# 21cmfast/21cmFAST

Hardware: AMD Instinct MI355X
Metric: IonizeBox cells/sec (512^3 HII_DIM, 40 filter radii) (higher is better)
Workload: dtype f32; 1 GPU; ComputeIonizedBox single-z, HII_DIM=512, 40 filter steps, G=2 (delta tophat + n_ion exp-MFP), first snapshot, device-resident inputs; hii_dim=512, n_radii=40, filtered_grids=2, parallelism=single GPU, fft=native

## Files before the change

### 21cmfast_amd/csrc/hip/c21hip.h

```cpp
#ifndef C21HIP_H
#define C21HIP_H

#include <stddef.h>

#include "ws_slots.h"

#ifdef __cplusplus
extern "C" {
#endif

int c21hip_device_count(void);
int c21hip_current_device(void);
int c21hip_use_device(int device);
int c21hip_is_device_ptr(const void *p);
void *c21hip_ws(int slot, size_t bytes);
__attribute__((visibility("hidden"))) const void *c21_stage_in(int slot, const void *p, size_t bytes, void *stream, int *status);
void *c21hip_ws_peek(int slot, size_t *bytes);
int c21hip_ws_adopt(int slot, void *ptr, size_t bytes);
void *c21hip_raw_alloc(size_t bytes);
void *c21hip_vmm_chunk(size_t phys_bytes, size_t map_bytes, void **va_out);
void c21hip_vmm_chunk_free(void *chunk);
int c21hip_ws_adopt_vmm(int slot, void *chunk, size_t bytes);
void c21hip_raw_free(void *p);
size_t c21hip_free_bytes(void);
// ... 59 lines not shown
                                 float R_param_a, const float *src_b, float *work_b,
                                 float *work_b2, int filter_b, float R_param_b, int nx, int ny,
                                 int nz, double box_len, double box_len_z, float R, float R2,
                                 int table_slot, int table_slot2, int phases, void *stream);
int c21hip_split_filter_x_pair1(const float *src, float *work, float *work2, int filter_type, int nx, int ny,
                                int nz, double box_len, double box_len_z, float R, float R2, int phases,
                                void *stream);
int c21hip_split_filter_xy2_pair_eval(const float *src_a, float *work_a, float *work_a2, int filter_a,
                                      const float *src_b, float *work_b, float *work_b2, int filter_b, int nx,
                                      int ny, int nz, double box_len, double box_len_z, float R, float R2,
                                      int phases, void *stream);
int c21hip_split_filter_xy_shared_pair(const float *src, float *work, float *work2,
                                       int filter_type, int nx, int ny, int nz, double box_len,
                                       double box_len_z, float R, float R2, int table_slot,
                                       int table_slot2, int phases, void *stream);
int c21hip_wev_prepare(int filter_a, float R_param_a, int filter_b, float R_param_b, int n_grids,
                       const float *R, int n_R, int nx, int ny, int nz, double box_len,
                       double box_len_z, int pair, int *enabled, void *stream);
void c21hip_wev_release(void);
int c21hip_wev_covers(void);
int c21hip_wev_applicable(int filter_a, int filter_b, int n_grids, int nx, int ny, int nz);
int c21hip_split_filter_xy_single_pair(const float *src, float *work, float *work2, int filter_type,
                                       float R_param, int nx, int ny, int nz, double box_len,
                                       double box_len_z, float R, float R2, int phases, void *stream);
typedef struct c21hip_z_ionise_desc {
    size_t size;
    const float *delta_work;
    const float *stars_work;
    const float *xe_work;
    const float *nrec_work;
    const float *nrec;
    double rec0;
    int recomb;
    float *g12;
    unsigned char *first_cross;
    unsigned *cross_plane;
    double *partials;
    double *sum_out;
    int nx, ny, nz, r_index;
    double rhocrit_omb, ion_eff;
    int mass_dep_zeta;
    double f_limit;
} c21hip_z_ionise_desc;
int c21hip_split_z_ionise(const c21hip_z_ionise_desc *desc, void *stream);
int c21hip_z_ionise_xe_supported(int nx, int ny, int nz);
int c21hip_z_ionise_recomb_supported(int nx, int ny, int nz);
int c21hip_z_ionise_recomb_xe_supported(int nx, int ny, int nz);
int c21hip_z_ionise_recomb_xe_nrec_supported(int nx, int ny, int nz);
int c21hip_z_ionise_partials(int nx, int ny, int nz);
int c21hip_split_z_sfr_gamma12(const float *sfr_work, const unsigned char *first_cross, float *g12,
                               int nx, int ny, int nz, int r_index, double g12_scale, void *stream);
int c21hip_z_xe_mask_supported(int nx, int ny, int nz);
int c21hip_split_z_xe_mask(const float *xe_work, const float *nion_dense, const double *mean_dev,
                           unsigned char *first_cross, int nx, int ny, int nz, int r_index,
                           double mean_f_coll, int fix_mean, int mass_dep_zeta, double f_limit,
                           double ion_eff, void *stream);
int c21hip_apply_first_cross_recomb(const unsigned char *first_cross, const float *R_dev,
                                    const float *prev_z_reion, int first_snapshot, double redshift,
                                    float *xH, float *z_reion, float *mfp, size_t ntot, void *stream);
int c21hip_window_tables(int table_slot, int filter_a, float R_param_a, int filter_b,
                         float R_param_b, int nx, int ny, int nz, double box_len,
                         double box_len_z, float R, void *stream);
int c21hip_split_z_c2r_minmax(const float *split_work, float *real_out, long out_zstride, int nx,
                              int ny, int nz, double *partials, double *minmax_out, void *stream);
int c21hip_z_table_band_supported(int nx, int ny, int nz);
int c21hip_split_z_minmax_only(const float *split_work, int nx, int ny, int nz, double *partials,
// ... 10 lines not shown
                             double *partials, double *stats_out, void *stream);
int c21hip_batched_stats(const double *partials, long stride, int nb, int count,
                         double *stats_out, void *stream);
int c21hip_floor_scale_stats(const float *in, long in_zstride, float *out, int nx, int ny, int nz,
                             double min_value, double const_factor, double *partials,
                             double *stats_out, void *stream);
int c21hip_split_z_c2r_div(const float *split_work, float *real_out, long out_zstride, int nx,
                           int ny, int nz, float divisor, void *stream);
int c21hip_split_z_c2r_out(const float *split_work, float *real_out, long out_zstride, int nx,
                           int ny, int nz, float scale, float divisor, int floor_density,
                           void *stream);
int c21hip_split_xblock_log2(int nx);
int c21hip_split_kop(const float *in_split, float *out_split, int nx, int ny, int nz,
                     double box_len, double box_len_z, int axis0, int axis1, void *stream);
int c21hip_split_sepop_xy(const float *split_src, float *split_work, int nx, int ny, int nz,
                          double box_len, double box_len_z, int axis0, int axis1, void *stream);
int c21hip_split_fold(const float *hi_split, float *lo_split, int nx, int ny, int nz, int f,
                      double box_len, double box_len_z, int axis0, int axis1, void *stream);
int c21hip_split_fold_multi(const float *hi_split, float *const lo_split[4], const int ops[4], int n_out, int nx,
                            int ny, int nz, int f, double box_len, double box_len_z, float tophat_R, void *stream);
int c21hip_lpt2_source(const float *const diag[3], const float *const off[3], float *out, size_t n,
                       float norm, void *stream);
int c21hip_copy_filter_split(const float *src_split, float *dst_split, int nx, int ny, int nz,
                             double box_len, double box_len_z, int filter_type, float R,
                             float R_param, int apply, void *stream);
int c21hip_split_z_c2r(const float *split_work, float *real_out, long out_zstride, int nx, int ny,
                       int nz, void *stream);
int c21hip_batched_means(const double *partials, long stride, int n_partials, int first, int step,
                         int count, double ntot, int mass_dep_zeta, double f_limit, double *sums,
                         double *means, void *stream);
int c21hip_z_cross_bits_supported(int nx, int ny, int nz);
int c21hip_resolve_crossings(const unsigned *bits, int r_hi, int r_lo, unsigned char *first_cross,
                             size_t nlines, void *stream);
int c21hip_split_filter_xy_shared(const float *src, float *work, int filter_type, int nx, int ny,
                                  int nz, double box_len, double box_len_z, float R, int apply,
                                  int table_slot, void *stream);
int c21hip_bench_pass(int kind, int n, int filter_a, int filter_b, float R, float R_param_b,
                      double box_len, int reps, void *stream, float *ms_out);
int c21hip_reduce_sum(const double *partials, int n, double *out, void *stream);
int c21hip_reduce_op(const double *partials, int n, int op, double *stage, double *out,
                     void *stream);

int c21hip_pack_clip(const float *dense, float *padded, int nx, int ny, int nz, double factor,
                     double lo, double hi, void *stream);
int c21hip_unpack_scale(const float *padded, float *dense, int nx, int ny, int nz, float scale,
                        void *stream);
int c21hip_divide_inplace(float *buf, size_t n, float divisor, void *stream);
int c21hip_divide_inplace_f64(float *buf, size_t n, double divisor, void *stream);
int c21hip_fill(float *buf, size_t n, float value, void *stream);
int c21hip_add_scalar(float *buf, size_t n, float value, void *stream);
int c21hip_widen(const float *in, double *out, size_t n, void *stream);

int c21hip_copy_filter(const float *src_c, float *dst_c, int nx, int ny, int nz, double box_len,
                       double box_len_z, int filter_type, float R, float R_param, int apply,
                       void *stream);
int c21hip_copy_filter_star(const float *src_c, float *dst_c, int nx, int ny, int nz,
                            double box_len, double box_len_z, int filter_type, float R,
                            float R_param, float R_star, int apply, void *stream);

typedef struct c21_gsl_stream_desc {
    unsigned long long out_offset;
    unsigned long long count;
    unsigned int kind;
    unsigned int state_offset;
} c21_gsl_stream_desc;
#define C21_GSL_HDR 8
// ... 537 lines not shown
```

### 21cmfast_amd/csrc/hip/fft_native.hip

```cpp
#include <hip/hip_runtime.h>

#include <cmath>
#include <map>
#include <mutex>
#include <vector>

#include "c21hip.h"
#include "fcoll_device.h"
#include "ms_window.h"
#include "c21cm_abi.h"
#include "c21cm_grid.h"

#ifndef C21X_XPAIR_THREADS
#define C21X_XPAIR_THREADS 512
#endif
#ifndef C21X_ZW_TSRC_OCC
#define C21X_ZW_TSRC_OCC 1
#endif
#ifndef C21X_ZW_BLOCK
#define C21X_ZW_BLOCK 256
#endif

namespace {
constexpr int kBlock = 256;
constexpr int TZ = 16;
constexpr int line_tile_cols(int n) { return n == 1536 ? TZ / 2 : TZ; }
template <int N>
__device__ __forceinline__ int fft_out_row(int g) {
    return (N >= 1024) ? ((g & 1) ? N / 2 + (g >> 1) : (g >> 1)) : g;
}

#ifndef C21X_XB_MIN
#define C21X_XB_MIN 1024
#endif
#ifndef C21X_XB_LOG2
#define C21X_XB_LOG2 3
#endif
__host__ __device__ constexpr int split_xb_log2(int nx) { return nx >= C21X_XB_MIN ? C21X_XB_LOG2 : 0; }
__host__ __device__ __forceinline__ long logical_line(long m, int ny, int lb) {
    if (lb == 0) return m;
    const long blk = (long)ny << lb;
    const long xbk = m / blk, rem = m - xbk * blk;
    const long y = rem >> lb, xi = rem & ((1 << lb) - 1);
    return ((xbk << lb) + xi) * ny + y;
}

#define LAUNCH_CHECK()                                                                  \
    do {                                                                                \
        hipError_t e_ = hipGetLastError();                                              \
        if (e_ != hipSuccess) {                                                         \
            c21hip_set_error("kernel launch failed: %s (%s:%d)", hipGetErrorString(e_), \
                             __FILE__, __LINE__);                                       \
            return C21CM_IO_ERROR;                                                      \
        }                                                                               \
    } while (0)

#include "fft_device.h"

template <int N, int COLS, int ROW, int R, int SIGN, bool LAST, int THREADS>
__device__ __forceinline__ void stockham_stage(float2 *tile, const float2 *tw, int log2s) {
    constexpr int NB = N / R;
    constexpr int ITEMS = NB * COLS;
    constexpr int kBlock = THREADS;
    constexpr int PER = (ITEMS + kBlock - 1) / kBlock;
    float2 v[PER][R];
#pragma unroll
    for (int u = 0; u < PER; u++) {
        const int i = threadIdx.x + kBlock * u;
        if (ITEMS % kBlock == 0 || i < ITEMS) {
            const int col = i % COLS, b = i / COLS;
#pragma unroll
// ... 1510 lines not shown
    __syncthreads();
    fft_tile<H, LZ, ZROW, -1, kBlock>(tile, twH);
    constexpr int NPRE = (H / 2 + 1) * LZ;
    for (int i = threadIdx.x; i < NPRE; i += kBlock) {
        const int li = i % LZ, k = i / LZ;
        if (k == 0) {
            const float2 z0 = tile[li];
            tile[li] = make_float2(z0.x + z0.y, 0.f);
            a.nyq[logical_line(l0 + li, a.ny, a.lb)] = make_float2(z0.x - z0.y, 0.f);
        } else {
            const float2 A = tile[k * ZROW + li], B = tile[(H - k) * ZROW + li];
            const float2 E = make_float2(0.5f * (A.x + B.x), 0.5f * (A.y - B.y));
            const float2 D = make_float2(0.5f * (A.x - B.x), 0.5f * (A.y + B.y));
            const float2 wD = cmul(D, twN[k]);
            tile[k * ZROW + li] = make_float2(E.x + wD.y, E.y - wD.x);
            tile[(H - k) * ZROW + li] = make_float2(E.x - wD.y, -E.y - wD.x);
        }
    }
    __syncthreads();
#pragma unroll
    for (int u = 0; u < NIN; u++) {
        const int f = threadIdx.x + kBlock * u;
        const int li = f / H, k = f % H;
        a.main[(l0 + li) * H + k] = tile[k * ZROW + li];
    }
}

struct ZFusedArgs {
    const float2 *d_main, *d_nyq;
    const float2 *s_main, *s_nyq;
    const float2 *x_main, *x_nyq;
    unsigned char *first_cross;
    unsigned *cross_bits;
    double *partials;
    double rhocrit_omb, ion_eff, f_limit;
    int mass_dep_zeta, r_index;
    int ny, lb;
    int store_all;
    int reverse;
    int rc;
    const float *nrec;
    double rec0;
    int x_is_nrec;
    const float2 *n_main, *n_nyq;
    float *g12;
};

template <int NZ>
__global__ void __launch_bounds__(kBlock)
z_c2r_ionise_kernel(ZFusedArgs a, const float2 *__restrict__ twH_global,
                    const float2 *__restrict__ twN_global) {
    constexpr int H = NZ / 2, LZ = LZ_FUSED, ZROW = LZ + 1;
    constexpr int NOUT = ZGeom<NZ, LZ>::NOUT;
    extern __shared__ float4 lds_raw[];
    float2 *tile = reinterpret_cast<float2 *>(lds_raw);
    float2 *twH = tile + H * ZROW;
    float2 *twN = twH + H;
    for (int t = threadIdx.x; t < H; t += kBlock) twH[t] = twH_global[t];
    for (int t = threadIdx.x; t <= H / 2; t += kBlock) twN[t] = twN_global[t];

    const long l0 = (long)blockIdx.x * LZ;
    float4 reg_d[ZGeom<NZ, LZ>::NLOAD], reg_s[ZGeom<NZ, LZ>::NLOAD];
    z_issue_loads<NZ, LZ>(a.d_main, l0, reg_d);
    z_issue_loads<NZ, LZ>(a.s_main, l0, reg_s);
    uchar2 old[NOUT];
#pragma unroll
// ... 473 lines not shown
            f1 = a.mass_dep_zeta && floor_lhs * opd1 > (opd1 + r1) * n1;
        }
        const bool i0 = (!RC && floor_ionises) || f0 || ((double)s0 * a.ion_eff > D0);
        const bool i1 = (!RC && floor_ionises) || f1 || ((double)s1 * a.ion_eff > D1);
        if constexpr (CB) {
            cb |= (i0 ? (1u << q) : 0u) | (i1 ? (0x10000u << q) : 0u);
            continue;
        }
        uchar2 m = MASK16 ? reinterpret_cast<const uchar2 *>(L)[j]
                          : (EARLY ? old[(EARLY && !MASK16) ? q : 0] : reinterpret_cast<const uchar2 *>(mrow)[j]);
        const bool n0 = i0 && m.x == 0, n1 = i1 && m.y == 0;
        if (n0) m.x = (unsigned char)a.r_index;
        if (n1) m.y = (unsigned char)a.r_index;
        if constexpr (MASK16) {
            if (n0 || n1) reinterpret_cast<uchar2 *>(L)[j] = m;
        } else if (n0 || n1 || a.store_all)
            reinterpret_cast<uchar2 *>(mrow)[j] = m;
        if constexpr (RC) {
            float *grow = a.g12 + lline * NZ + 2 * j;
            if (n0 && a.rc != 2) grow[0] = fmaxf(xd[q].x, dmin);
            if (n1 && a.rc != 2) grow[1] = fmaxf(xd[q].y, dmin);
        }
        if constexpr (TS && RC) __builtin_amdgcn_sched_barrier(0);
    }
    if constexpr (MASK16) {
        wave_fence();
#pragma unroll
        for (int v = 0; v < MV; v++) {
            const uint4 n = reinterpret_cast<const uint4 *>(L)[b * MV + v], o = mreg[v];
            if (a.store_all || n.x != o.x || n.y != o.y || n.z != o.z || n.w != o.w)
                reinterpret_cast<uint4 *>(mrow)[b * MV + v] = n;
        }
    }
    if constexpr (CB) a.cross_bits[lline * (NZ / 32) + b] = cb;
#pragma unroll
    for (int off = 32; off > 0; off >>= 1) acc += __shfl_down(acc, off, 64);
    if (lane == 0) red[wave] = acc;
    __syncthreads();
    if (threadIdx.x == 0) {
        double sum = 0.;
#pragma unroll
        for (int w = 0; w < ZBLK / 64; w++) sum += red[w];
        a.partials[blk] = sum;
    }
}

template <int A, int EPI, int P = 16>
__global__ void __launch_bounds__(kBlock)
zw_c2r_kernel(ZPassArgs a, const float2 *__restrict__ twH_global,
              const float2 *__restrict__ twN_global) {
    constexpr int H = P * A, NZ = 2 * H, ZWL = zw_lines(P);
    constexpr int LINE_LDS = A * (P + 1) + 4;
    static_assert(LINE_LDS % 2 == 0, "16-byte aligned line regions (EPI 7)");
    __shared__ __attribute__((aligned(16))) float2 lines[ZWL * LINE_LDS];
    __shared__ float2 twH[H], twN[H];
    for (int t = threadIdx.x; t < H; t += kBlock) {
        twH[t] = twH_global[t];
        twN[t] = twN_global[t];
    }
    const int lane = threadIdx.x & 63, wave = threadIdx.x >> 6;
    const int g = lane / P, b = lane % P;
    const int lw = wave * (64 / P) + g;
    const unsigned blk = a.reverse ? gridDim.x - 1 - blockIdx.x : blockIdx.x;
    const long line = (long)blk * ZWL + lw;
    float2 *L = lines + lw * LINE_LDS;
    const float2 *src = a.main + line * H;
    float2 x[A];
// ... 1747 lines not shown
}

extern "C" int c21hip_split_z_ionise(const c21hip_z_ionise_desc *d, void *stream) {
    if (!d || d->size != sizeof(*d)) {
        c21hip_set_error("fused pass Z: the descriptor's size member is not sizeof(c21hip_z_ionise_desc)");
        return C21CM_VALUE_ERROR;
    }
    if (d->cross_plane && !c21hip_z_cross_bits_supported(d->nx, d->ny, d->nz)) {
        c21hip_set_error("fused pass Z: crossing bits are not available for this grid");
        return C21CM_VALUE_ERROR;
    }
    const long nlines = (long)d->nx * d->ny;
    const long n_main = nlines * (d->nz / 2);
    const ZFusedWant w{d->xe_work != nullptr, d->recomb != 0, d->recomb && d->nrec_work, d->cross_plane != nullptr};
    ZFusedArgs a{};
    a.ny = d->ny;
    a.lb = split_xb_log2(d->nx);
    a.d_main = reinterpret_cast<const float2 *>(d->delta_work);
    a.d_nyq = a.d_main + n_main;
    a.s_main = reinterpret_cast<const float2 *>(d->stars_work);
    a.s_nyq = a.s_main + n_main;
    const float *third = w.xe ? d->xe_work : (w.nrec ? d->nrec_work : nullptr);
    if (third) {
        a.x_main = reinterpret_cast<const float2 *>(third);
        a.x_nyq = a.x_main + n_main;
    }
    if (w.xe && w.nrec) {
        a.n_main = reinterpret_cast<const float2 *>(d->nrec_work);
        a.n_nyq = a.n_main + n_main;
    } else
        a.x_is_nrec = w.nrec;
    a.first_cross = d->first_cross;
    a.cross_bits = d->cross_plane;
    a.partials = d->partials;
    a.rhocrit_omb = d->rhocrit_omb;
    a.ion_eff = d->ion_eff;
    a.f_limit = d->f_limit;
    a.mass_dep_zeta = d->mass_dep_zeta;
    a.r_index = d->r_index;
    if (w.rc) {
#ifdef C21CM_DIAG_BUILD
        a.rc = getenv("C21CM_DIAG_RC_NOSTORE") ? 2 : 1;
#else
        a.rc = 1;
#endif
        a.g12 = d->g12;
        if (!w.nrec) {
            a.nrec = d->nrec;
            a.rec0 = d->rec0;
        }
        a.reverse = 1;
    } else {
        static const int store_all = [] {
            const char *e = getenv("C21CM_MASK_STORE_ALL");
            return (e && e[0] == '1') ? 1 : 0;
        }();
        a.store_all = store_all;
        static const int reverse = [] {
            const char *e = getenv("C21CM_ZREV");
            return (e && e[0] == '0') ? 0 : 1;
        }();
        a.reverse = reverse;
    }
    int n_partials = 0;
    const int st = dispatch_z_fused(d->nz, a, w, nlines, (hipStream_t)stream, &n_partials);
    if (st || w.rc || !d->sum_out) return st;
// ... 222 lines not shown
        if (kind == 8) {
            pair2[0] = (float *)c21hip_ws(WS_BENCH_A2, nf * sizeof(float));
            pair2[1] = (float *)c21hip_ws(WS_BENCH_B2, nf * sizeof(float));
            if (!pair2[0] || !pair2[1]) return C21CM_MEMORY_ALLOC_ERROR;
        }
    }
    hipEvent_t e0, e1;
    if (hipEventCreate(&e0) != hipSuccess || hipEventCreate(&e1) != hipSuccess)
        return C21CM_IO_ERROR;
    for (int r = -2; r < reps && !st; r++) {
        if (r == 0) (void)hipEventRecord(e0, stream);
        if (kind == 0 || kind == 7)
            st = filter_xy(src, work, 2, n, n, n, box_len, box_len, ft, R, rp, 1, stream_, 2);
        else if (kind == 8)
            st = filter_xy_pair(a, real, pair2[0], filter_a, 0.f, b, real2, pair2[1], filter_b,
                                R_param_b, n, n, n, box_len, box_len, R, 0.9f * R, 0, 1, 2,
                                stream_);
        else if (kind == 1)
            st = filter_xy(src, work, 2, n, n, n, box_len, box_len, ft, R, rp, 1, stream_, 4);
        else if (kind == 4)
            st = filter_xy(src, work, 2, n, n, n, box_len, box_len, ft, R, rp, 1, stream_, 1);
        else if (kind == 6)
            st = filter_xy_pair(a, real, pair2[0], filter_a, 0.f, b, real2, pair2[1], filter_b,
                                R_param_b, n, n, n, box_len, box_len, R, 0.9f * R, 0, 1, 2,
                                stream_);
        else if (kind == 5)
            st = filter_xy(src, work, 2, n, n, n, box_len, box_len, ft, R, rp, 0, stream_, 2);
        else if (kind == 2) {
            c21hip_z_ionise_desc d{};
            d.size = sizeof(d);
            d.delta_work = a;
            d.stars_work = b;
            if (c21hip_z_cross_bits_supported(n, n, n))
                d.cross_plane = reinterpret_cast<unsigned *>(mask);
            else
                d.first_cross = mask;
            d.partials = partials;
            d.sum_out = partials + nlines / 4 + 40;
            d.nx = d.ny = d.nz = n;
            d.r_index = 5;
            d.rhocrit_omb = 6.2e9;
            d.ion_eff = 1.0;
            d.mass_dep_zeta = 1;
            d.f_limit = 1e-9;
            st = c21hip_split_z_ionise(&d, stream);
        } else
            st = dispatch_z_c2r(n, z_pass_base(a, real, n + 2, n, n, n), nlines, stream);
    }
    (void)hipEventRecord(e1, stream);
    (void)hipEventSynchronize(e1);
    float ms = 0.f;
    (void)hipEventElapsedTime(&ms, e0, e1);
    (void)hipEventDestroy(e0);
    (void)hipEventDestroy(e1);
    *ms_out = ms / (float)reps;
    if (kind == 7 || kind == 8) c21hip_wev_release();
    return st;
}

extern "C" int c21hip_native_fft_c2r(float *padded, int nx, int ny, int nz, void *stream) {
    const size_t bytes = c21hip_split_floats(nx, ny, nz) * sizeof(float);
    float *split = (float *)c21hip_ws(WS_NATIVE_C2R_SPLIT, bytes);
    if (!split) return C21CM_MEMORY_ALLOC_ERROR;
    int st = c21hip_padded_to_split(padded, split, nx, ny, nz, stream);
    if (st) return st;
    return c21hip_split_filter_c2r(split, split, padded, 2 * (long)(nz / 2 + 1), nx, ny, nz, 1.0,
                                   1.0, 0, 0.f, 0.f, 0, stream);
// ... 3 lines not shown
```

### 21cmfast_amd/csrc/hip/ionize_kernels.hip

```cpp
#include <hip/hip_runtime.h>

#include <cmath>
#include <cstdint>

#include "c21hip.h"
#include "c21cm_abi.h"
#include "c21cm_grid.h"
#include "fcoll_device.h"

namespace {
constexpr int kBlock = 256;
constexpr int kMaxBlocks = 256 * 8;
constexpr double kTiny = 1e-30;
constexpr double kMinDensityLowLimit = 9e-8;

inline int grid_for(size_t work_items) {
    size_t b = (work_items + kBlock - 1) / kBlock;
    if (b > (size_t)kMaxBlocks) b = kMaxBlocks;
    if (b < 1) b = 1;
    return (int)b;
}

#define LAUNCH_CHECK()                                                                  \
    do {                                                                                \
        hipError_t e_ = hipGetLastError();                                              \
        if (e_ != hipSuccess) {                                                         \
            c21hip_set_error("kernel launch failed: %s (%s:%d)", hipGetErrorString(e_), \
                             __FILE__, __LINE__);                                       \
            return C21CM_IO_ERROR;                                                      \
        }                                                                               \
    } while (0)

__device__ __forceinline__ double wave_sum(double v) {
#pragma unroll
    for (int off = 32; off > 0; off >>= 1) v += __shfl_down(v, off, 64);
    return v;
}
__device__ __forceinline__ double wave_min(double v) {
#pragma unroll
    for (int off = 32; off > 0; off >>= 1) v = fmin(v, __shfl_down(v, off, 64));
    return v;
// ... 1008 lines not shown
                    res_xH -= x_e;
                    if (res_xH < 0)
                        res_xH = 0;
                    else if (res_xH > 1)
                        res_xH = 1;
                    x = (float)res_xH;
                }
                acc_x += (double)x;
                if (!a.minimize_memory) {
                    if (zr > 0.f && (double)x < kTiny) {
                        T = fully_ionized_T(zr, stored_z, dens, pow_Tre, pow_z);
                        if (T < T_neutral) T = T_neutral;
                    }
                    if (!isfinite(T)) bad = 1;
                }
                xo.v[e] = x;
                zo.v[e] = zr;
                To.v[e] = T;
            }
            xo.store(xH, i);
            zo.store(z_reion, i);
            if (!a.minimize_memory) To.store(Tk, i);
        }
    }
    if (bad) atomicOr(flag, 1);
    block_sum_to(acc_s, partials_stars + chunk0);
    __syncthreads();
    block_sum_to(acc_x, partials_xh + chunk0);
}

template <int NS>
__global__ void __launch_bounds__(kBlock)
resolve_crossings_kernel(const unsigned *__restrict__ bits, size_t plane_words, int r_hi, int r_lo,
                         unsigned char *__restrict__ first_cross, size_t nquads) {
    const size_t t = (size_t)blockIdx.x * kBlock + threadIdx.x;
    if (t >= nquads) return;
    unsigned seen[4] = {0u, 0u, 0u, 0u}, sl[NS][4];
#pragma unroll
    for (int s = 0; s < NS; s++)
#pragma unroll
        for (int i = 0; i < 4; i++) sl[s][i] = 0u;
#pragma unroll 4
    for (int r = r_hi; r >= r_lo; r--) {
        const uint4 w = reinterpret_cast<const uint4 *>(bits + (size_t)(r - 1) * plane_words)[t];
        const unsigned wv[4] = {w.x, w.y, w.z, w.w};
#pragma unroll
        for (int i = 0; i < 4; i++) {
            const unsigned fresh = wv[i] & ~seen[i];
            seen[i] |= wv[i];
#pragma unroll
            for (int s = 0; s < NS; s++)
                if ((r >> s) & 1) sl[s][i] |= fresh;
        }
    }
    unsigned char *row = first_cross + (t >> 2) * 512 + 8 * (t & 3);
#pragma unroll
    for (int q = 0; q < 16; q++) {
        unsigned v[4];
#pragma unroll
        for (int i = 0; i < 4; i++) {
            v[i] = 0u;
#pragma unroll
            for (int s = 0; s < NS; s++) v[i] |= ((sl[s][i] >> q) & 0x00010001u) << s;
        }
        uint2 o;
        o.x = (v[0] & 0xffu) | ((v[0] >> 16) << 8) | ((v[1] & 0xffu) << 16) | ((v[1] >> 16) << 24);
        o.y = (v[2] & 0xffu) | ((v[2] >> 16) << 8) | ((v[3] & 0xffu) << 16) | ((v[3] >> 16) << 24);
        *reinterpret_cast<uint2 *>(row + 32 * q) = o;
    }
}

__global__ void __launch_bounds__(kBlock)
apply_first_cross_kernel(const unsigned char *__restrict__ fc,
                         const float *__restrict__ prev_z_reion, int first_snapshot, float z_now,
                         float *__restrict__ xH, float *__restrict__ z_reion, size_t ntot) {
    for (size_t i = (size_t)blockIdx.x * kBlock + threadIdx.x; i < ntot;
         i += (size_t)gridDim.x * kBlock) {
        if (fc[i]) {
            const float pz = first_snapshot ? -1.f : prev_z_reion[i];
            z_reion[i] = (pz < 0.f) ? z_now : pz;
            xH[i] = 0.f;
        }
    }
}

__global__ void __launch_bounds__(kBlock)
apply_first_cross_recomb_kernel(const unsigned char *__restrict__ fc, const float *__restrict__ R_dev,
                                const float *__restrict__ prev_z_reion, int first_snapshot,
// ... 700 lines not shown
    return 0;
}

extern "C" int c21hip_final_sweep_eulerian(const c21hip_ionize_args *a, double stored_redshift,
                                           const unsigned char *first_cross, const float *nion_dense,
                                           const double *mean_dev, const float *density,
                                           const float *prev_z_reion, float *xH, float *z_reion,
                                           float *kinetic_temperature, double *partials, double *sum_xh_out,
                                           int *flag_out, const float *xe_dense,
                                           const float *kinetic_temp_neutral, void *stream) {
    const int st = c21hip_final_sweep_eulerian_range(a, stored_redshift, first_cross, nion_dense, mean_dev,
                                                     density, prev_z_reion, xH, z_reion, kinetic_temperature,
                                                     partials, flag_out, xe_dense, kinetic_temp_neutral, 0, -1,
                                                     stream);
    if (st) return st;
    return c21hip_final_sweep_reduce(a, 1, partials, nullptr, sum_xh_out, stream);
}

extern "C" int c21hip_brightness_temp(const float *density, const float *xH, const float *Ts,
                                      float *bt, float *tau, size_t n, float const_factor,
                                      float T_rad, double redshift, int use_ts, double *partials,
                                      double *sum_out, void *stream) {
    const int blocks = grid_for(n);
    hipLaunchKernelGGL(brightness_kernel, dim3(blocks), dim3(kBlock), 0, (hipStream_t)stream,
                       density, xH, Ts, bt, tau, n, const_factor, T_rad, redshift, use_ts,
                       partials);
    LAUNCH_CHECK();
    hipLaunchKernelGGL(finish_reduce_kernel, dim3(1), dim3(kBlock), 0, (hipStream_t)stream,
                       partials, blocks, 0, sum_out);
    LAUNCH_CHECK();
    return 0;
}

extern "C" int c21hip_resolve_crossings(const unsigned *bits, int r_hi, int r_lo,
                                        unsigned char *first_cross, size_t nlines, void *stream) {
    if (r_lo < 1 || r_hi > 255 || !nlines) {
        c21hip_set_error("resolve_crossings: radius indices 1..255 and at least one line");
        return C21CM_VALUE_ERROR;
    }
    const size_t nquads = nlines * 4;
    const dim3 grid((unsigned)((nquads + kBlock - 1) / kBlock));
    if (r_hi < 64)
        hipLaunchKernelGGL(resolve_crossings_kernel<6>, grid, dim3(kBlock), 0, (hipStream_t)stream, bits,
                           nlines * 16, r_hi, r_lo, first_cross, nquads);
    else
        hipLaunchKernelGGL(resolve_crossings_kernel<8>, grid, dim3(kBlock), 0, (hipStream_t)stream, bits,
                           nlines * 16, r_hi, r_lo, first_cross, nquads);
    LAUNCH_CHECK();
    return 0;
}

extern "C" int c21hip_apply_first_cross(const unsigned char *first_cross,
                                        const float *prev_z_reion, int first_snapshot,
                                        double redshift, float *xH, float *z_reion, size_t ntot,
                                        void *stream) {
    hipLaunchKernelGGL(apply_first_cross_kernel, dim3(grid_for(ntot)), dim3(kBlock), 0,
                       (hipStream_t)stream, first_cross, prev_z_reion, first_snapshot,
                       (float)redshift, xH, z_reion, ntot);
    LAUNCH_CHECK();
    return 0;
}

extern "C" int c21hip_apply_first_cross_recomb(const unsigned char *first_cross, const float *R_dev,
                                               const float *prev_z_reion, int first_snapshot,
                                               double redshift, float *xH, float *z_reion,
                                               float *mfp, size_t ntot, void *stream) {
    hipLaunchKernelGGL(apply_first_cross_recomb_kernel, dim3(grid_for(ntot)), dim3(kBlock), 0,
                       (hipStream_t)stream, first_cross, R_dev, prev_z_reion, first_snapshot,
                       (float)redshift, xH, z_reion, mfp, ntot);
    LAUNCH_CHECK();
    return 0;
}

template <typename T>
__global__ void __launch_bounds__(kBlock)
max_into_kernel(T *__restrict__ dst, const T *__restrict__ src, size_t n) {
    for (size_t i = (size_t)blockIdx.x * kBlock + threadIdx.x; i < n; i += (size_t)gridDim.x * kBlock)
        dst[i] = src[i] > dst[i] ? src[i] : dst[i];
}

extern "C" int c21hip_max_into(void *dst, const void *src, size_t count, int bytes_per_element,
                               void *stream) {
// ... 541 lines not shown
```

### 21cmfast_amd/csrc/host/ionize_driver.c

```c
#include <math.h>
#include <stdio.h>
#include <stdlib.h>
#include <string.h>

#include "../hip/c21hip.h"
#include "c21cm_grid.h"

#define MAX_COPYBACK 12
typedef struct {
    void *host[MAX_COPYBACK];
    void *dev[MAX_COPYBACK];
    size_t bytes[MAX_COPYBACK];
    int n;
} copyback_list;

#define SC_SUMS 0
#define SC_MEANS (SC_SUMS + C21CM_MAX_RADII)
#define SC_MINMAX (SC_MEANS + C21CM_MAX_RADII)
#define SC_XHSUM (SC_MINMAX + 4)
#define SC_FLAG (SC_XHSUM + 1)
#define SC_G12SUM (SC_FLAG + 1)
#define SC_SUMS_M (SC_G12SUM + 1)
#define SC_MEANS_M (SC_SUMS_M + C21CM_MAX_RADII)
#define SC_MINMAX_M (SC_MEANS_M + C21CM_MAX_RADII)
// ... 636 lines not shown
    return 0;
}

static int z_ionise_radius(ion_ctx *c, int R_ct, const float *dwork, const float *swork,
                           const float *xwork, unsigned char *first_cross) {
    int status = 0;
    const c21cm_ionize_spec *s = c->s;
    double *sum_dev = c->scalars + SC_SUMS + R_ct;
    c21hip_z_ionise_desc d = {.size = sizeof(d), .delta_work = dwork, .stars_work = swork,
                              .recomb = c->fused_rc, .first_cross = first_cross, .partials = c->partials,
                              .nx = c->nx, .ny = c->ny, .nz = c->nz, .r_index = R_ct,
                              .rhocrit_omb = s->rhocrit_omb, .ion_eff = s->ion_eff_factor,
                              .mass_dep_zeta = s->mass_dep_zeta, .f_limit = s->f_limit_acg};
    if (c->def_partials) {
        TRY(defer_radius(c, R_ct));
        d.partials = c->def_partials + (long)R_ct * c->def_stride;
    } else if (!c->fused_rc)
        d.sum_out = sum_dev;
    if (c->fused_rc) {
        d.g12 = c->G12;
        if (c->x4_on) {
            d.xe_work = c->cur_xe;
            d.nrec_work = c->cur_x4;
        } else if (c->x3_nrec)
            d.nrec_work = c->cur_xe;
        else {
            d.xe_work = s->use_ts_fluct ? c->cur_xe : NULL;
            d.nrec = c->inhomo ? c->prev_nrec : NULL;
            d.rec0 = c->rec0;
        }
    } else if (c->cross_bits) {
        d.first_cross = NULL;
        d.cross_plane = c->cross_bits + (size_t)(R_ct - 1) * (c->ntot / 32);
    } else
        d.xe_work = xwork;
    TRY(c21hip_split_z_ionise(&d, c->stream));
    if (c->fused_rc)
        TRY(c21hip_split_z_sfr_gamma12(xwork, first_cross, c->G12, c->nx, c->ny, c->nz, R_ct,
                                       s->R[R_ct] * s->gamma_prefactor, c->stream));
    if (!c->def_partials) {
        if (c->fused_rc)
            TRY(c21hip_reduce_sum(d.partials, c21hip_z_ionise_partials(c->nx, c->ny, c->nz), sum_dev, c->stream));
        TRY(c21hip_finish_mean(sum_dev, (double)c->ntot, s->mass_dep_zeta, s->f_limit_acg,
                               c->scalars + SC_MEANS + R_ct, c->stream));
    }
done:
    return status;
}

static int fused_step(ion_ctx *c, int R_a, int R_b, unsigned char *first_cross, int next_a,
                      int next_b) {
    int status = 0;
    const c21cm_ionize_spec *s = c->s;
    const int set = c->tab_seq & 1;
    const int buf_a = 2 * set, buf_b = 2 * set + 1;
    tab_init();
    const int tab_async = !c->wev && g_tab.enabled && c->ntot >= ((size_t)1 << 26);
    if (tab_async) {
        if (c->tab_seq == 0) {
            TRY(c21hip_event_record(g_tab.ev_sync, c->stream));
            TRY(c21hip_stream_wait_event(g_tab.aux, g_tab.ev_sync));
            TRY(tab_build_async(c, R_a, buf_a));
            if (R_b >= 1) TRY(tab_build_async(c, R_b, buf_b));
        }
        if (next_a >= 1) TRY(tab_build_async(c, next_a, 2 * (set ^ 1)));
        if (next_b >= 1) TRY(tab_build_async(c, next_b, 2 * (set ^ 1) + 1));
// ... 1178 lines not shown
        return;
    c->cross_bits = (unsigned *)c21hip_ws(WS_CROSS_BITS, (size_t)(s->n_radii - 1) * (c->ntot / 8));
}

int c21cm_ionize_grids(const c21cm_ionize_spec *spec, const PerturbedField *perturbed_field,
                       const IonizedBox *previous_ionize_box, const TsBox *spin_temp,
                       const HaloBox *halos, IonizedBox *box, c21cm_ionize_report *report,
                       void *stream) {
    int status = validate_spec(spec, perturbed_field, halos, spin_temp, box);
    if (status) return status;
    ion_ctx c;
    phase_clock clk = {{NULL}, 0, 0};
    unsigned char *mask = NULL;
    g_spectra.valid = 0;
    TRY(ctx_setup(&c, spec, perturbed_field, previous_ionize_box, spin_temp, halos, box, 1, 1, stream));
    TRY(clock_start(&clk, 4, stream));
    TRY(init_output_grids(&c, previous_ionize_box));
    TRY(preloop(&c));
    TRY(clock_mark(&clk, stream));
    if (c.fused || c.eul_mask || c.sphere) {
        mask = (unsigned char *)c21hip_ws(WS_FIRST_CROSS, c.ntot);
        if (!mask) {
            status = C21CM_MEMORY_ALLOC_ERROR;
            goto done;
        }
        cross_bits_begin(&c);
        if (!c.cross_bits)
            TRY(c21hip_memset(mask, 0, c.ntot, stream));
    }
    TRY(native_wev_prepare(&c));
    if (mask) {
        TRY(radii_ladder(&c, spec->n_radii - 1, 1, mask, spec->r_lowest == 0 ? 0 : -1));
        if (c.cross_bits) {
            TRY(c21hip_resolve_crossings(c.cross_bits, spec->n_radii - 1, spec->r_lowest > 1 ? spec->r_lowest : 1,
                                         mask, (size_t)c.nx * c.ny, stream));
            c.cross_bits = NULL;
        }
        TRY(flush_deferred(&c));
        TRY(c.fused_rc ? finish_first_cross_recomb(&c, mask) : finish_first_cross(&c, mask, 0));
    } else {
        for (int R_ct = spec->n_radii - 1; R_ct >= spec->r_lowest; R_ct--)
            TRY(one_radius(&c, R_ct, NULL, -1));
        TRY(flush_deferred(&c));
    }
    c21hip_wev_release();
    TRY(clock_mark(&clk, stream));
    TRY(postloop(&c, box, report));
    TRY(clock_mark(&clk, stream));
    if (report) {
        report->ms_preloop = clock_ms(&clk, 0);
        report->ms_rloop = clock_ms(&clk, 1);
        report->ms_postloop = clock_ms(&clk, 2);
    }
done:
    c21hip_wev_release();
    clock_free(&clk);
    return status;
}

static int no_mini_shards(void) {
    c21hip_set_error("ionize: the sharded R loop does not take USE_MINI_HALOS");
    return C21CM_VALUE_ERROR;
}

static struct {
    int valid, n;
    double means[C21CM_MAX_RADII];
} g_shard_means;
// ... 520 lines not shown
```

### 21cmfast_amd/csrc/host/perturb_driver.c

```c
#include <math.h>
#include <stdlib.h>
#include <string.h>

#include "../hip/c21hip.h"
#include "c21cm_grid.h"

#define L_FACTOR 0.620350491

_Static_assert(WS_PT_IN_LAST - WS_PT_IN0 == 6 && WS_PT_OUT_LAST - WS_PT_OUT0 == 3 &&
                   WS_PT_SPLIT_LAST - WS_PT_SPLIT == 2,
               "perturb: staging slot ranges");

static int pt_split_supported(const int lo_dim[3]) {
    const char *e = getenv("C21CM_PT");
    if (e && e[0] == 'p') return 0;
    return c21hip_fft_is_native(lo_dim[0], lo_dim[1], lo_dim[2]) &&
           !c21hip_split_xblock_log2(lo_dim[0]);
}

#define TRY(expr)         \
    do {                  \
        int st_ = (expr); \
        if (st_) {        \
            status = st_; \
            goto done;    \
        }                 \
    } while (0)

int c21cm_perturb_grids(const c21cm_perturb_spec *s, const InitialConditions *ics,
                        PerturbedField *pf, void *stream) {
    int status = 0;
    if (!s || !ics || !pf || !pf->density) {
        c21hip_set_error("perturb: NULL spec / ics / density");
        return C21CM_VALUE_ERROR;
    }
    if (s->hii_dim < 2 || s->dim < s->hii_dim) {
        c21hip_set_error("perturb: bad dimensions DIM=%d HII_DIM=%d", s->dim, s->hii_dim);
        return C21CM_VALUE_ERROR;
    }
    const int lo_dim[3] = {s->hii_dim, s->hii_dim, s->hii_dim_z};
    const int hi_dim[3] = {s->dim, s->dim, s->dim_z};
    const int hires = s->perturb_on_high_res;
    const int *box_dim = hires ? hi_dim : lo_dim;
    const int linear = (s->perturb_algorithm == C21CM_PERTURB_LINEAR);
    const int lpt2 = (s->perturb_algorithm == C21CM_PERTURB_2LPT);
    const size_t lo_tot = (size_t)lo_dim[0] * lo_dim[1] * lo_dim[2];
    const size_t hi_tot = (size_t)hi_dim[0] * hi_dim[1] * hi_dim[2];
    const size_t lo_npad = (size_t)lo_dim[0] * lo_dim[1] * 2 * (size_t)(lo_dim[2] / 2 + 1);
    const size_t hi_npad = (size_t)hi_dim[0] * hi_dim[1] * 2 * (size_t)(hi_dim[2] / 2 + 1);
    const size_t b_tot = hires ? hi_tot : lo_tot;
// ... 160 lines not shown
```

Baseline: 3.464 billion cells/s.

## Enable x-blocked split layout at 512^3 and index crossing bits by memory line

```diff
diff --git a/21cmfast_amd/csrc/hip/c21hip.h b/21cmfast_amd/csrc/hip/c21hip.h
--- a/21cmfast_amd/csrc/hip/c21hip.h
+++ b/21cmfast_amd/csrc/hip/c21hip.h
@@ -115,6 +115,7 @@
     const float *nrec;
     double rec0;
     int recomb;
+    int cross_by_memory_line;
     float *g12;
     unsigned char *first_cross;
     unsigned *cross_plane;
@@ -191,6 +192,8 @@
 int c21hip_z_cross_bits_supported(int nx, int ny, int nz);
 int c21hip_resolve_crossings(const unsigned *bits, int r_hi, int r_lo, unsigned char *first_cross,
                              size_t nlines, void *stream);
+int c21hip_resolve_crossings_lines(const unsigned *bits, int r_hi, int r_lo, unsigned char *first_cross,
+                                   size_t nlines, int ny, int lb, void *stream);
 int c21hip_split_filter_xy_shared(const float *src, float *work, int filter_type, int nx, int ny,
                                   int nz, double box_len, double box_len_z, float R, int apply,
                                   int table_slot, void *stream);
diff --git a/21cmfast_amd/csrc/hip/fft_native.hip b/21cmfast_amd/csrc/hip/fft_native.hip
--- a/21cmfast_amd/csrc/hip/fft_native.hip
+++ b/21cmfast_amd/csrc/hip/fft_native.hip
@@ -30,13 +30,19 @@
     return (N >= 1024) ? ((g & 1) ? N / 2 + (g >> 1) : (g >> 1)) : g;
 }
 
-#ifndef C21X_XB_MIN
-#define C21X_XB_MIN 1024
-#endif
-#ifndef C21X_XB_LOG2
-#define C21X_XB_LOG2 3
-#endif
-__host__ __device__ constexpr int split_xb_log2(int nx) { return nx >= C21X_XB_MIN ? C21X_XB_LOG2 : 0; }
+constexpr int kXb512Default = 4;
+static int split_xb_log2(int nx) {
+    if (nx >= 1024) return 3;
+    if (nx < 512) return 0;
+    static const int k512 = [] {
+        const char *e = getenv("C21CM_XBLOCK");
+        if (!e || !*e) return kXb512Default;
+        char *end = nullptr;
+        const long k = strtol(e, &end, 10);
+        return (*end == 0 && (k == 0 || (k >= 3 && k <= 5))) ? (int)k : kXb512Default;
+    }();
+    return k512;
+}
 __host__ __device__ __forceinline__ long logical_line(long m, int ny, int lb) {
     if (lb == 0) return m;
     const long blk = (long)ny << lb;
@@ -1613,6 +1619,7 @@
     const float2 *x_main, *x_nyq;
     unsigned char *first_cross;
     unsigned *cross_bits;
+    int cb_mem;
     double *partials;
     double rhocrit_omb, ion_eff, f_limit;
     int mass_dep_zeta, r_index;
@@ -2152,7 +2159,7 @@
                 reinterpret_cast<uint4 *>(mrow)[b * MV + v] = n;
         }
     }
-    if constexpr (CB) a.cross_bits[lline * (NZ / 32) + b] = cb;
+    if constexpr (CB) a.cross_bits[(a.cb_mem ? line : lline) * (NZ / 32) + b] = cb;
 #pragma unroll
     for (int off = 32; off > 0; off >>= 1) acc += __shfl_down(acc, off, 64);
     if (lane == 0) red[wave] = acc;
@@ -3966,6 +3973,7 @@
         a.x_is_nrec = w.nrec;
     a.first_cross = d->first_cross;
     a.cross_bits = d->cross_plane;
+    a.cb_mem = d->cross_by_memory_line;
     a.partials = d->partials;
     a.rhocrit_omb = d->rhocrit_omb;
     a.ion_eff = d->ion_eff;
@@ -4254,7 +4262,7 @@
             d.delta_work = a;
             d.stars_work = b;
             if (c21hip_z_cross_bits_supported(n, n, n))
-                d.cross_plane = reinterpret_cast<unsigned *>(mask);
+                d.cross_plane = reinterpret_cast<unsigned *>(mask), d.cross_by_memory_line = 1;
             else
                 d.first_cross = mask;
             d.partials = partials;
diff --git a/21cmfast_amd/csrc/hip/ionize_kernels.hip b/21cmfast_amd/csrc/hip/ionize_kernels.hip
--- a/21cmfast_amd/csrc/hip/ionize_kernels.hip
+++ b/21cmfast_amd/csrc/hip/ionize_kernels.hip
@@ -7,6 +7,7 @@
 #include "c21cm_abi.h"
 #include "c21cm_grid.h"
 #include "fcoll_device.h"
+#include "split_layout.h"
 
 namespace {
 constexpr int kBlock = 256;
@@ -1081,7 +1082,7 @@
 template <int NS>
 __global__ void __launch_bounds__(kBlock)
 resolve_crossings_kernel(const unsigned *__restrict__ bits, size_t plane_words, int r_hi, int r_lo,
-                         unsigned char *__restrict__ first_cross, size_t nquads) {
+                         unsigned char *__restrict__ first_cross, size_t nquads, int ny, int lb) {
     const size_t t = (size_t)blockIdx.x * kBlock + threadIdx.x;
     if (t >= nquads) return;
     unsigned seen[4] = {0u, 0u, 0u, 0u}, sl[NS][4];
@@ -1102,7 +1103,7 @@
                 if ((r >> s) & 1) sl[s][i] |= fresh;
         }
     }
-    unsigned char *row = first_cross + (t >> 2) * 512 + 8 * (t & 3);
+    unsigned char *row = first_cross + (size_t)c21_logical_line((long)(t >> 2), ny, lb) * 512 + 8 * (t & 3);
 #pragma unroll
     for (int q = 0; q < 16; q++) {
         unsigned v[4];
@@ -1869,22 +1870,31 @@
     return 0;
 }
 
-extern "C" int c21hip_resolve_crossings(const unsigned *bits, int r_hi, int r_lo,
-                                        unsigned char *first_cross, size_t nlines, void *stream) {
+extern "C" int c21hip_resolve_crossings_lines(const unsigned *bits, int r_hi, int r_lo, unsigned char *first_cross,
+                                              size_t nlines, int ny, int lb, void *stream) {
     if (r_lo < 1 || r_hi > 255 || !nlines) {
         c21hip_set_error("resolve_crossings: radius indices 1..255 and at least one line");
+        return C21CM_VALUE_ERROR;
+    }
+    if (lb < 0 || lb > 8 || (lb > 0 && (ny < 1 || nlines % ((size_t)ny << lb)))) {
+        c21hip_set_error("resolve_crossings: %zu lines are not whole blocks of %d x 2^%d lines", nlines, ny, lb);
         return C21CM_VALUE_ERROR;
     }
     const size_t nquads = nlines * 4;
     const dim3 grid((unsigned)((nquads + kBlock - 1) / kBlock));
     if (r_hi < 64)
         hipLaunchKernelGGL(resolve_crossings_kernel<6>, grid, dim3(kBlock), 0, (hipStream_t)stream, bits,
-                           nlines * 16, r_hi, r_lo, first_cross, nquads);
+                           nlines * 16, r_hi, r_lo, first_cross, nquads, ny, lb);
     else
         hipLaunchKernelGGL(resolve_crossings_kernel<8>, grid, dim3(kBlock), 0, (hipStream_t)stream, bits,
-                           nlines * 16, r_hi, r_lo, first_cross, nquads);
-    LAUNCH_CHECK();
-    return 0;
+                           nlines * 16, r_hi, r_lo, first_cross, nquads, ny, lb);
+    LAUNCH_CHECK();
+    return 0;
+}
+
+extern "C" int c21hip_resolve_crossings(const unsigned *bits, int r_hi, int r_lo,
+                                        unsigned char *first_cross, size_t nlines, void *stream) {
+    return c21hip_resolve_crossings_lines(bits, r_hi, r_lo, first_cross, nlines, 1, 0, stream);
 }
 
 extern "C" int c21hip_apply_first_cross(const unsigned char *first_cross,
diff --git a/21cmfast_amd/csrc/host/ionize_driver.c b/21cmfast_amd/csrc/host/ionize_driver.c
--- a/21cmfast_amd/csrc/host/ionize_driver.c
+++ b/21cmfast_amd/csrc/host/ionize_driver.c
@@ -692,6 +692,7 @@
     } else if (c->cross_bits) {
         d.first_cross = NULL;
         d.cross_plane = c->cross_bits + (size_t)(R_ct - 1) * (c->ntot / 32);
+        d.cross_by_memory_line = 1;
     } else
         d.xe_work = xwork;
     TRY(c21hip_split_z_ionise(&d, c->stream));
@@ -1936,8 +1937,9 @@
     if (mask) {
         TRY(radii_ladder(&c, spec->n_radii - 1, 1, mask, spec->r_lowest == 0 ? 0 : -1));
         if (c.cross_bits) {
-            TRY(c21hip_resolve_crossings(c.cross_bits, spec->n_radii - 1, spec->r_lowest > 1 ? spec->r_lowest : 1,
-                                         mask, (size_t)c.nx * c.ny, stream));
+            TRY(c21hip_resolve_crossings_lines(c.cross_bits, spec->n_radii - 1, spec->r_lowest > 1 ? spec->r_lowest : 1,
+                                               mask, (size_t)c.nx * c.ny, c.ny, c21hip_split_xblock_log2(c.nx),
+                                               stream));
             c.cross_bits = NULL;
         }
         TRY(flush_deferred(&c));
diff --git a/21cmfast_amd/csrc/host/perturb_driver.c b/21cmfast_amd/csrc/host/perturb_driver.c
--- a/21cmfast_amd/csrc/host/perturb_driver.c
+++ b/21cmfast_amd/csrc/host/perturb_driver.c
@@ -14,8 +14,7 @@
 static int pt_split_supported(const int lo_dim[3]) {
     const char *e = getenv("C21CM_PT");
     if (e && e[0] == 'p') return 0;
-    return c21hip_fft_is_native(lo_dim[0], lo_dim[1], lo_dim[2]) &&
-           !c21hip_split_xblock_log2(lo_dim[0]);
+    return c21hip_fft_is_native(lo_dim[0], lo_dim[1], lo_dim[2]) && lo_dim[0] < 1024;
 }
 
 #define TRY(expr)         \
```

Result: faster. 3.575 billion cells/s, median of 6 (+3.2%).
